# brantburnett/Snappier

Measured on AMD Instinct MI355X. Metric: uncompressed GB/s block compress+decompress, 64 KiB blocks, higher is better.
Workload: dtype u8

## Files before the change

snappier_amd/csrc/capi_internal.h:

```cpp
#pragma once
#include <hip/hip_runtime.h>

#include <cstdio>
#include <cstring>
#include <new>
#include <algorithm>
#include <cmath>
#include <chrono>
#include <mutex>
#include <string>
#include <utility>
#include <vector>

#include "snp_rules.h"

struct ChunkRows {
    u8* type;
    u64 *body_off, *out_off;
    u32 *body_len, *crc, *out_cap, *out_len, *tag;
    i32* status;
};

extern "C" {
hipError_t snp_launch_decompress(const u8*, const u64*, const u32*, u32, u8*, const u64*, const u32*, u32*, i32*,
                                 const u8*, int, hipStream_t, const u32*);
u32 snp_tag_index_entries(u32, u32);
size_t snp_tag_index_workspace_bytes(u32, u32);
size_t snp_tag_index_fallback_offset(u32, u32);
hipError_t snp_launch_tag_index(const u8*, u32, u32, u32, u64*, u64*, u32*, u64*, u32*, u32*, hipStream_t);
u32 snp_tag_index_chunks_ready(u32, u32, u64);
hipError_t snp_launch_tag_index_begin(u64*, u32, u32, int, hipStream_t);
int snp_tag_index_look_back_only(u32, u32);
hipError_t snp_launch_tag_index_chunks(const u8*, u32, u32, u64*, u32, u32, hipStream_t);
hipError_t snp_launch_tag_index_finish(const u8*, u32, u32, u32, u64*, u64*, u32*, u64*, u32*, u32*, hipStream_t);
hipError_t snp_launch_compress_win(const u8*, const u64*, const u32*, u32, u8*, const u64*, u32*, i32*, int, int, int,
                                   hipStream_t, uint16_t*, u32);
size_t snp_compress_win_table_bytes(u32);
hipError_t snp_launch_compress_win_dual(const u8*, const u64*, const u32*, u32, u8*, const u64*, u32*, i32*, int, int, hipStream_t, hipStream_t,
                                        hipEvent_t, hipEvent_t, uint16_t*, u32, u32, u32*);
hipError_t snp_launch_decompress_small(const u8*, const u64*, const u32*, u32, u8*, const u64*, const u32*, u32*, i32*, const u8*,
                                       u32, hipStream_t, u32*, u32*, u32, u32);
hipError_t snp_launch_sample_caps(const u32*, u32, u32, u32*, hipStream_t);
hipError_t snp_launch_decompress_list(const u8*, const u64*, const u32*, u32, u8*, const u64*, const u32*, u32*, i32*, const u8*, int,
                                      hipStream_t, const u32*, u32*, u32, u32);
hipError_t snp_launch_compress_lanes(const u8*, const u64*, const u32*, u32, u8*, const u64*, u32*, i32*, int, int, const snp_table_pieces*,
                                     u32*, hipStream_t, const snp_lane_tuning*);
size_t snp_compress_lanes_workspace(u32);
hipError_t snp_probe_tables(const snp_table_pieces*, u32, u32, hipStream_t, float*);
hipError_t snp_launch_crc32c(const u8*, const u64*, const u32*, u32, int, u32*, const u32*, i32*, hipStream_t);
hipError_t snp_launch_gather(const u8*, const u64*, const u32*, u8*, const u64*, u32, hipStream_t);
hipError_t snp_launch_frame_chunks(u64, u32, u64, u64*, u32*, u64*, hipStream_t);
hipError_t snp_launch_frame_plan(const u32*, const u32*, u32, u8*, u32*, u64*, u64*, hipStream_t);
hipError_t snp_launch_frame_header_only(u8*, u64*, hipStream_t);
hipError_t snp_launch_frame_scan(const u8*, u64, u64, u32, const ChunkRows&, u64*, hipStream_t);
hipError_t snp_launch_frame_result(const i32*, const u64*, u64*, hipStream_t);
size_t snp_frame_scan_workspace(u64);
hipError_t snp_launch_frame_scan_spans(const u8*, u64, u64, u32, const ChunkRows&, u64*, void*, hipStream_t);
hipError_t snp_launch_frame_emit(const u8*, const u64*, const u8*, const u64*, const u8*, const u32*, const u32*,
                                 const u64*, u8*, u64, u32, hipStream_t);
}

constexpr u64 snp_comp_stride(u64 n) { return (38 + n + n / 6 + 15) / 16 * 16 + 16; }
constexpr u64 kSnpCompStride = snp_comp_stride(SNP_BLOCK_SIZE);
static_assert(kSnpCompStride == 76496 + 16, "staging stride of a 64 KiB fragment");

struct DevBuf {
    void* p = nullptr;
    size_t cap = 0;
};

inline u64 snp_align_up(u64 v, u64 a) { return (v + a - 1) / a * a; }

struct TablePool {
    std::mutex mu;
    int users = 0;
    snp_table_pieces tp{};
    void* plain = nullptr;
    size_t plain_cap = 0;
    std::vector<void*> pieces;
    hipEvent_t last_use = nullptr;
    hipStream_t last_stream = nullptr;
    bool used = false;
    bool pinned = false;
    std::vector<void*> retired;
    uint64_t stats[4] = {0, 0, 0, 0};
    void drain();
    void drop_workspace();
    void destroy();
};
TablePool* snp_pool_of(int device);
constexpr int kSnpMaxDevices = 64;

struct RelaxedCaptureMode {
    hipStreamCaptureMode mode = hipStreamCaptureModeRelaxed;
    bool ok;
    RelaxedCaptureMode() { ok = hipThreadExchangeStreamCaptureMode(&mode) == hipSuccess; if (!ok) (void)hipGetLastError(); }
    ~RelaxedCaptureMode() { if (ok && hipThreadExchangeStreamCaptureMode(&mode) != hipSuccess) (void)hipGetLastError(); }
};

struct snp_ctx {
    int device = 0;
    int variant = SNP_HASH_CRC32C;
    hipStream_t stream = nullptr;
    bool own_stream = false;
    int fenced = 0;
    int dec_lds = 0;
    int decode_layout = 0;
    int table_tries = 2;
    uint64_t table_probe_max_bytes = 0;
    u32 par_min = 4 * SNP_BLOCK_SIZE;
    int compress_mode = 0;
    int win_np = 1;
    u32 small_max = 512;
    u32 small_min_blocks = 4096;
    int crc_kernel = 0;
    int crc_bits() const { return crc_kernel == 1 ? 2 : crc_kernel == 2 ? 4 : 0; }
    bool no_prepass = false;
    bool small_lanes = false;
    bool redo_grid = false, redo_list = false;
    u32 small_team_log = 0;
    u32 slice_fragments = 262144;
    u32 win_gtab_min = 4096;
    u32 win_gslots = 0;
    u32 win_dual_min = 1536;
    hipStream_t side_stream = nullptr;
    hipEvent_t side_ev[2] = {nullptr, nullptr};
    int side_state = 0;
    bool side_stream_ready();
    u32 win_max = 32768;
    snp_lane_tuning lane_tune{0, -1, 0, -1, 0, 0};
    DevBuf in, out, meta, work, fragtab, scan, small, redo, win_tables;
    int frame_scan = 0;
    uint64_t counters[7] = {0, 0, 0, 0, 0, 0, 0};
    bool table_tries_set = false;
    std::string err;

    bool launch_decompress(const u8* d_in, const u64* in_off, const u32* in_len, u32 nblocks, u8* d_out, const u64* out_off,
                           const u32* out_cap, u32* out_len, i32* status, const u8* chunk_type);
    bool launch_compress(const u8* d_in, const u64* in_off, const u32* in_len, u32 nblocks, u8* d_out, const u64* out_off,
                         u32* out_len, i32* status, int emit_varint);
    bool decode_chunks(const u8* d_in, const ChunkRows& r, u32 n, u8* d_out);
    u32* hint = nullptr;
    hipEvent_t hint_ev = nullptr;
    bool hint_pending = false, hint_mostly_large = false, hint_from_prepass = false, hint_seen = false;
    u32 hint_blocks = 0, hint_mean_cap = 256;
    bool hint_ready();
    u32 n_waves = 0;
    u32 persistent_waves();
    u32* chint = nullptr;
    hipEvent_t chint_ev = nullptr;
    bool chint_pending = false, chint_small = false, chint_mid = false;
    int chint_tiny = 0;
    bool chint_ready();

    bool check(hipError_t e, const char* what);
    bool ensure(DevBuf& b, size_t bytes, const char* what);
    bool h2d(void* dev, const void* host, size_t n, const char* what);
    bool d2h(void* host, const void* dev, size_t n, const char* what);
    bool stream_is_capturing();
    bool was_captured = false;
    std::vector<void*> kept;
    bool use_device() { return check(hipSetDevice(device), "hipSetDevice"); }
    bool rebind(hipStream_t next);
    hipEvent_t order_ev = nullptr;
    hipStream_t copy_stream = nullptr;
    hipEvent_t copy_ev[2] = {nullptr, nullptr};
    int copy_state = 0;
    bool copy_stream_ready();

    TablePool* pool = nullptr;
    snp_table_pieces tp{};
    bool borrowed = false;
    DevBuf own_tables;
    bool borrow_tables(u32 nblocks, bool thorough = false);
    void return_tables();
    bool build_tables(TablePool& P, u32 nblocks, bool thorough, bool capturing);

    bool upload_and_compress(const u8* host_in, size_t n, u32 nf, const u64* d_in_off, const u32* d_in_len, u8* d_out,
                             const u64* d_out_off, u32* d_out_len, i32* d_status, int emit_varint);
};

struct DevGuard {
    int prev = -1, dev = -1;
    bool ok = false;
    explicit DevGuard(snp_ctx* c) : dev(c->device)
    {
        if (hipGetDevice(&prev) != hipSuccess) prev = -1;
        ok = prev == dev || c->use_device();
        if (ok && !c->was_captured && c->stream) (void)c->stream_is_capturing();
    }
    ~DevGuard() { if (prev >= 0 && prev != dev) (void)hipSetDevice(prev); }
};

snp_status snp_frame_encode_impl(snp_ctx* c, const uint8_t* d_in, const uint8_t* host_in, uint64_t n, uint8_t* d_out, uint64_t cap,
                                 uint64_t* d_written, void* d_work);
inline bool snp_ranges_overlap(const u8* a, size_t an, const u8* b, size_t bn) { return an && bn && a < b + bn && b < a + an; }
```

snappier_amd/csrc/capi_pool.hip:

```cpp
#include "capi_internal.h"
#include "piece_search.h"

using snp_piece_search::PieceSearch;

void TablePool::drain()
{
    RelaxedCaptureMode relaxed;
    if (used && last_use) (void)hipEventSynchronize(last_use);
}

void TablePool::drop_workspace()
{
    drain();
    RelaxedCaptureMode relaxed;
    auto gone = [&](void* q) { if (!q) return; if (pinned) retired.push_back(q); else (void)hipFree(q); };
    gone(plain);
    for (void* q : pieces) gone(q);
    plain = nullptr;
    plain_cap = 0;
    pieces.clear();
    tp = snp_table_pieces{};
}

void TablePool::destroy()
{
    pinned = false;
    drop_workspace();
    for (void* q : retired) (void)hipFree(q);
    retired.clear();
    if (last_use) (void)hipEventDestroy(last_use);
    last_use = nullptr;
    used = false;
}

namespace {
std::mutex g_pools_mu;
}
TablePool* snp_pool_of(int device)
{
    static TablePool* pools[kSnpMaxDevices] = {};
    if (device < 0 || device >= kSnpMaxDevices) return nullptr;
    std::lock_guard<std::mutex> g(g_pools_mu);
    if (!pools[device]) pools[device] = new TablePool();
    return pools[device];
}

bool snp_ctx::borrow_tables(u32 nblocks, bool thorough)
{
    if (table_tries_set && table_tries == 1) {
        const size_t bytes = snp_compress_lanes_workspace(nblocks);
        if (bytes > own_tables.cap) {
            if (stream_is_capturing()) { err = "hash-table workspace: it would have to grow while the stream is being captured"; return false; }
            (void)hipStreamSynchronize(stream);
            if (own_tables.p) { if (was_captured) kept.push_back(own_tables.p); else (void)hipFree(own_tables.p); }
            own_tables = DevBuf{};
            if (!check(hipMalloc(&own_tables.p, bytes + 4096), "hipMalloc(hash tables)")) { own_tables.p = nullptr; return false; }
            own_tables.cap = bytes + 4096;
        }
        tp = snp_table_pieces{};
        tp.p[0] = static_cast<u32*>(own_tables.p);
        tp.piece_frags = 0xffffffc0u;
        tp.n = 1;
        counters[2] = counters[3] = counters[4] = counters[5] = 0;
        return true;
    }
    TablePool& P = *pool;
    P.mu.lock();
    const bool capturing = stream_is_capturing();
    if (!build_tables(P, nblocks, thorough, capturing)) { P.mu.unlock(); return false; }
    if (capturing) {
        P.pinned = true;
    } else if (P.used && P.last_stream != stream) {
        if (!check(hipStreamWaitEvent(stream, P.last_use, 0), "hipStreamWaitEvent(table pool)")) { P.mu.unlock(); return false; }
    }
    tp = P.tp;
    counters[2] = P.stats[0]; counters[3] = P.stats[1]; counters[4] = P.stats[2]; counters[5] = P.stats[3];
    borrowed = true;
    return true;
}

void snp_ctx::return_tables()
{
    if (!borrowed) return;
    TablePool& P = *pool;
    if (!stream_is_capturing()) {
        if (!P.last_use && hipEventCreateWithFlags(&P.last_use, hipEventDisableTiming) != hipSuccess) { (void)hipGetLastError(); P.last_use = nullptr; }
        if (P.last_use && hipEventRecord(P.last_use, stream) == hipSuccess) { P.used = true; P.last_stream = stream; }
        else { (void)hipGetLastError(); (void)hipStreamSynchronize(stream); P.used = false; }
    }
    borrowed = false;
    P.mu.unlock();
}

bool snp_ctx::build_tables(TablePool& P, u32 nblocks, bool thorough, bool capturing)
{
    const size_t bytes = snp_compress_lanes_workspace(nblocks);
    if (!P.pieces.empty() && static_cast<uint64_t>(nblocks) <= static_cast<uint64_t>(P.tp.piece_frags) * P.tp.n) return true;
    if (P.pieces.empty() && P.plain && bytes <= P.plain_cap) return true;
    if (capturing) {
        err = "hash-table workspace: it would have to be built while the stream is being captured -- call snp_ctx_reserve_compress (or make the same call once) before the capture";
        return false;
    }
    RelaxedCaptureMode relaxed;
    const int tries = table_tries_set ? table_tries : 2;
    P.drop_workspace();
    P.stats[0] = P.stats[1] = P.stats[2] = P.stats[3] = 0;
    if (bytes < (1ull << 30) || tries <= 1) {
        const size_t want = bytes >= (1ull << 30) ? bytes + 4096 : bytes + bytes / 4 + 4096;
        if (!check(hipMalloc(&P.plain, want), "hipMalloc(hash tables)")) { P.plain = nullptr; return false; }
        P.plain_cap = want;
        P.tp = snp_table_pieces{};
        P.tp.p[0] = static_cast<u32*>(P.plain);
        P.tp.piece_frags = 0xffffffc0u;
        P.tp.n = 1;
        return true;
    }
    PieceSearch ps{};
    const uint64_t with_slack = static_cast<uint64_t>(nblocks) + nblocks / 16u;
    const u32 cap_frags = static_cast<u32>(with_slack < slice_fragments ? with_slack : (nblocks > slice_fragments ? nblocks : slice_fragments));
    const u32 piece_frags = ((cap_frags + SNP_TABLE_PIECES_MAX - 1) / SNP_TABLE_PIECES_MAX + 63u) / 64u * 64u;
    const size_t piece_bytes = static_cast<size_t>(piece_frags) * 65536u;
    ps.n = (cap_frags + piece_frags - 1) / piece_frags;
    ps.piece_gib = piece_bytes / 1073741824.0;
    ps.max_cand = static_cast<size_t>(ps.n) * static_cast<size_t>(tries);
    ps.dbg = SNP_GETENV("SNAPPIER_HIP_DEBUG") != nullptr;
    if (thorough && table_tries_set) ps.patience = 64;
    size_t free_b = 0, total_b = 0;
    if (hipMemGetInfo(&free_b, &total_b) == hipSuccess) {
        size_t room = free_b / 2;
        if (table_probe_max_bytes) {
            room = static_cast<size_t>(table_probe_max_bytes);
            if (room > free_b / 8 * 7) room = free_b / 8 * 7;
        }
        if (room / piece_bytes < ps.max_cand) ps.max_cand = room / piece_bytes;
    }
    if (ps.max_cand < ps.n) ps.max_cand = ps.n;
    std::vector<u32*> cand;
    ps.alloc_one = [&]() {
        void* q = nullptr;
        if (hipMalloc(&q, piece_bytes) != hipSuccess) { (void)hipGetLastError(); return false; }
        cand.push_back(static_cast<u32*>(q));
        return true;
    };
    ps.probe_set = [&](const std::vector<u32>& pick) {
        snp_table_pieces t{};
        for (size_t i = 0; i < pick.size(); ++i) t.p[i] = cand[pick[i]];
        t.piece_frags = piece_frags;
        t.n = static_cast<u32>(pick.size());
        float ms = 1e30f;
        if (snp_probe_tables(&t, nblocks, 512u, stream, &ms) != hipSuccess) { (void)hipGetLastError(); ms = 1e30f; }
        return ms;
    };
    std::vector<u32> set;
    const auto t_search = std::chrono::steady_clock::now();
    const float ms = ps.run(set);
    if (ms < 0) {
        for (u32* q : cand) (void)hipFree(q);
        err = "hipMalloc(hash tables): out of memory";
        return false;
    }
    std::vector<char> used(cand.size(), 0);
    P.tp = snp_table_pieces{};
    for (u32 i = 0; i < ps.n; ++i) { P.tp.p[i] = cand[set[i]]; used[set[i]] = 1; P.pieces.push_back(cand[set[i]]); }
    P.tp.piece_frags = piece_frags;
    P.tp.n = ps.n;
    for (size_t k = 0; k < cand.size(); ++k)
        if (!used[k]) (void)hipFree(cand[k]);
    P.stats[0] = ms < 1e6f ? static_cast<uint64_t>(ms * 1000.0f) : 0;
    P.stats[1] = static_cast<uint64_t>(cand.size());
    P.stats[2] = static_cast<uint64_t>(std::chrono::duration_cast<std::chrono::microseconds>(std::chrono::steady_clock::now() - t_search).count());
    P.stats[3] = static_cast<uint64_t>(cand.size()) * piece_bytes;
    return true;
}
```

snappier_amd/csrc/compress_lanes.hip:

```cpp
#include <cstdlib>

#include "snp_device.h"

#ifndef SNP_CL_FLAT
#define SNP_CL_FLAT 1
#endif
#ifndef SNP_CL_SLOTS
#define SNP_CL_SLOTS 1
#endif

namespace {

constexpr u32 kDefaultSlots = SNP_CL_SLOTS;

constexpr u32 crc_step32(u32 x)
{
    for (int k = 0; k < 32; ++k) x = (x >> 1) ^ ((x & 1u) ? 0x82F63B78u : 0u);
    return x;
}

__device__ __forceinline__ u32 check_bits(u32 bytes) { return (bytes * 0x9E3779B1u) & 0xffff0000u; }

__device__ __forceinline__ u32 table_swap(u32* p, u32 v) { return __hip_atomic_exchange(p, v, __ATOMIC_RELAXED, __HIP_MEMORY_SCOPE_AGENT); }

struct LaneCtx {
    const u8* src;
    u8* dst;
    u32* table;
    u32 first4;
    u32 n;
    u32 mask;
    u32 hmask;
};

template <int VARIANT>
__device__ __forceinline__ u32 lane_hash(const LaneCtx& c, u32 bytes, const u16 (*lut)[256])
{
    u32 hash;
    if constexpr (VARIANT == SNP_HASH_CRC32C) {
        hash = lut[0][bytes & 0xffu] ^ lut[1][(bytes >> 8) & 0xffu] ^ lut[2][(bytes >> 16) & 0xffu] ^ lut[3][bytes >> 24] ^ c.hmask;
    } else {
        hash = (0x1e35a7bdu * bytes) >> 17;
    }
    return (hash & c.mask) >> 1;
}

__device__ __forceinline__ u32 lane_emit_literal(const LaneCtx& c, u32 op, u32 s, u32 len)
{
    u8* o = c.dst + op;
    const u32 k = len - 1;
    u32 hdr;
    if (k < 60) { o[0] = static_cast<u8>(k << 2); hdr = 1; }
    else if (k < 256) { o[0] = static_cast<u8>(60u << 2); o[1] = static_cast<u8>(k); hdr = 2; }
    else { o[0] = static_cast<u8>(61u << 2); o[1] = static_cast<u8>(k); o[2] = static_cast<u8>(k >> 8); hdr = 3; }
    const u8* src = c.src + s;
    u8* d = o + hdr;
    u32 i = 0;
    for (; i + 16 <= len; i += 16)
        *reinterpret_cast<snp_u128_unaligned*>(d + i) = *reinterpret_cast<const snp_u128_unaligned*>(src + i);
    for (; i + 4 <= len; i += 4) st32u(d + i, ld32u(src + i));
    for (; i < len; ++i) d[i] = src[i];
    return op + hdr + len;
}

__device__ __forceinline__ u32 lane_emit_literal16(const LaneCtx& c, u32 op, u32 s, u32 len, const snp_u128_unaligned& first, u32 cap, bool merge)
{
    u8* o = c.dst + op;
    const u32 k = len - 1;
    if (merge && len <= 15 && op + 16 <= cap) {
        snp_u128_unaligned w;
        w.v[0] = (first.v[0] << 8) | (k << 2);
        w.v[1] = __builtin_amdgcn_alignbit(first.v[1], first.v[0], 24);
        w.v[2] = __builtin_amdgcn_alignbit(first.v[2], first.v[1], 24);
        w.v[3] = __builtin_amdgcn_alignbit(first.v[3], first.v[2], 24);
        *reinterpret_cast<snp_u128_unaligned*>(o) = w;
        return op + 1 + len;
    }
    u32 hdr;
    if (k < 60) { o[0] = static_cast<u8>(k << 2); hdr = 1; }
    else if (k < 256) { o[0] = static_cast<u8>(60u << 2); o[1] = static_cast<u8>(k); hdr = 2; }
    else { o[0] = static_cast<u8>(61u << 2); o[1] = static_cast<u8>(k); o[2] = static_cast<u8>(k >> 8); hdr = 3; }
    u8* d = o + hdr;
    if (len >= 16 || op + hdr + 16 <= cap) {
        *reinterpret_cast<snp_u128_unaligned*>(d) = first;
    } else {
        u32 w[4] = {first.v[0], first.v[1], first.v[2], first.v[3]};
        u32 at = 0, wi = 0;
        if (len & 8) { st32u(d, w[0]); st32u(d + 4, w[1]); at = 8; wi = 2; }
        if (len & 4) { st32u(d + at, w[wi]); at += 4; ++wi; }
        u32 rest = w[wi & 3];
        if (len & 2) { d[at] = static_cast<u8>(rest); d[at + 1] = static_cast<u8>(rest >> 8); rest >>= 16; at += 2; }
        if (len & 1) d[at] = static_cast<u8>(rest);
    }
    if (len > 16) {
        const u8* src = c.src + s;
        u32 i = 16;
        for (; i + 16 <= len; i += 16)
            *reinterpret_cast<snp_u128_unaligned*>(d + i) = *reinterpret_cast<const snp_u128_unaligned*>(src + i);
        if (i < len)
            *reinterpret_cast<snp_u128_unaligned*>(d + len - 16) = *reinterpret_cast<const snp_u128_unaligned*>(src + len - 16);
    }
    return op + hdr + len;
}

__device__ __forceinline__ u32 lane_emit_copy64(u8* dst, u32 op, u32 off, u32 len, u32 cap)
{
    u8* o = dst + op;
    const bool one = len < 12 && off < 2048;
    const u32 w = one ? (1u | ((len - 4) << 2) | ((off >> 8) << 5) | ((off & 0xffu) << 8)) : (2u | ((len - 1) << 2) | (off << 8));
    if (op + 4 <= cap) {
        st32u(o, w);
    } else {
        o[0] = static_cast<u8>(w);
        o[1] = static_cast<u8>(w >> 8);
        if (!one) o[2] = static_cast<u8>(w >> 16);
    }
    return op + (one ? 2u : 3u);
}

__device__ __forceinline__ u32 lane_emit_copy(u8* dst, u32 op, u32 off, u32 len, u32 cap = 0)
{
    while (len >= 68) { op = lane_emit_copy64(dst, op, off, 64, cap); len -= 64; }
    if (len > 64) { op = lane_emit_copy64(dst, op, off, 60, cap); len -= 60; }
    return lane_emit_copy64(dst, op, off, len, cap);
}

__device__ __forceinline__ u32 lane_find_match_length(const u8* src, u32 s1, u32 s2, u32 n)
{
    u32 matched = 0;
    while (s2 + matched + 8 <= n) {
        const u64 x = ld64u(src + s1 + matched) ^ ld64u(src + s2 + matched);
        if (x) return matched + (static_cast<u32>(__builtin_ctzll(x)) >> 3);
        matched += 8;
    }
    while (s2 + matched < n && src[s1 + matched] == src[s2 + matched]) ++matched;
    return matched;
}

constexpr u32 kStageStride = 100;

struct OutStage {
    u8* lds;
    u32 flushed;
};

__device__ __forceinline__ void stage_flush64(const LaneCtx& c, OutStage& st)
{
    u8* g = c.dst + st.flushed;
    typedef u32 v4u __attribute__((ext_vector_type(4), aligned(1)));
#pragma unroll
    for (u32 i = 0; i < 64; i += 16) {
        const snp_u128_unaligned q = *reinterpret_cast<const snp_u128_unaligned*>(st.lds + i);
        const v4u v = {q.v[0], q.v[1], q.v[2], q.v[3]};
        __builtin_nontemporal_store(v, reinterpret_cast<v4u*>(g + i));
    }
    const snp_u128_unaligned t0 = *reinterpret_cast<const snp_u128_unaligned*>(st.lds + 64);
    const snp_u128_unaligned t1 = *reinterpret_cast<const snp_u128_unaligned*>(st.lds + 80);
    *reinterpret_cast<snp_u128_unaligned*>(st.lds) = t0;
    *reinterpret_cast<snp_u128_unaligned*>(st.lds + 16) = t1;
    st.flushed += 64;
}

__device__ __forceinline__ void stage_drain(const LaneCtx& c, OutStage& st, u32 op)
{
    const u32 fill = op - st.flushed;
    u8* g = c.dst + st.flushed;
    u32 i = 0;
    for (; i + 16 <= fill; i += 16)
        *reinterpret_cast<snp_u128_unaligned*>(g + i) = *reinterpret_cast<const snp_u128_unaligned*>(st.lds + i);
    for (; i < fill; ++i) g[i] = st.lds[i];
    st.flushed = op;
}

enum : int {
    kOptBlindLiterals = 1,
    kOptBlindLiteral16 = 2,
    kOptBlindCopies = 4,
    kOptShortExtend = 8,
    kOptStagedOutput = 16,
    kOptExchangeProbe = 64,
    kOptInputWindow = 128,
};

template <int VARIANT, u32 kSlots, bool SMALL>
__global__ __launch_bounds__(SNP_WAVE) void k_compress_lanes(const u8* __restrict__ in, const u64* __restrict__ in_off,
                                                            const u32* __restrict__ in_len, u32 nblocks,
                                                            u8* __restrict__ out, const u64* __restrict__ out_off,
                                                            u32* __restrict__ out_len, i32* __restrict__ status,
                                                            int emit_varint, const snp_table_pieces tp, int opts,
                                                            const u32* __restrict__ max_len, u32 small_max)
{
    __shared__ u16 lut[4][256];
    if (VARIANT == SNP_HASH_CRC32C) {
        for (u32 e = threadIdx.x; e < 1024; e += blockDim.x)
            lut[e >> 8][e & 255u] = static_cast<u16>(crc_step32((e & 255u) << (8 * (e >> 8))) & 0x7ffeu);
        __syncthreads();
    }
    __shared__ u8 s_out[SMALL ? 16 : SNP_WAVE * kStageStride];
    const u32 b = blockIdx.x * blockDim.x + threadIdx.x;
    const u32 maxlen = *max_len;
    if (SMALL ? maxlen > small_max : (small_max != 0 && maxlen <= small_max)) return;
    extern __shared__ __attribute__((aligned(16))) u8 s_dyn[];
    const u32 tstride = maxlen > 16384 ? 16384u : maxlen < 256 ? 256u : (2u << (31u - __clz(maxlen - 1)));
    u32* wt;
    {
        const u32 first = blockIdx.x * blockDim.x;
        const u32 mine = nblocks - first < blockDim.x ? nblocks - first : blockDim.x;
        const u32 piece = first / tp.piece_frags;
        wt = tp.p[piece] + static_cast<size_t>(first - piece * tp.piece_frags) * tstride;
        const size_t words = static_cast<size_t>(mine) * tstride;
        if (tstride == 16384u) {
            typedef u32 v4u __attribute__((ext_vector_type(4)));
            const v4u zero4 = {0, 0, 0, 0};
            for (size_t i = static_cast<size_t>(threadIdx.x) * 4; i < words; i += static_cast<size_t>(blockDim.x) * 4)
                __builtin_nontemporal_store(zero4, reinterpret_cast<v4u*>(wt + i));
        } else {
            for (size_t i = static_cast<size_t>(threadIdx.x) * 4; i < words; i += static_cast<size_t>(blockDim.x) * 4)
                *reinterpret_cast<uint4*>(wt + i) = make_uint4(0, 0, 0, 0);
        }
        asm volatile("s_waitcnt vmcnt(0)" ::: "memory");
    }
    if (b >= nblocks) return;
    const bool staged = (opts & kOptStagedOutput) != 0;
    const bool t_swap = kSlots == 1 && (opts & kOptExchangeProbe) != 0;
    bool in_win = (opts & kOptInputWindow) != 0;
    OutStage stg{(SMALL ? s_dyn + blockDim.x * (small_max + 16u) : s_out) + threadIdx.x * kStageStride, 0};

    LaneCtx c;
    c.dst = out + out_off[b];
    c.n = in_len[b];
    c.table = wt + static_cast<size_t>(threadIdx.x) * tstride;
    const u32 n = c.n;
    if constexpr (SMALL) {
        const u8* g = in + in_off[b];
        u8* mine = s_dyn + threadIdx.x * (small_max + 16u);
        u32 i = 0;
        for (; i + 16 <= n; i += 16) {
            const snp_u128_unaligned q = *reinterpret_cast<const snp_u128_unaligned*>(g + i);
            *reinterpret_cast<uint4*>(mine + i) = make_uint4(q.v[0], q.v[1], q.v[2], q.v[3]);
        }
        for (; i + 4 <= n; i += 4) *reinterpret_cast<u32*>(mine + i) = ld32u(g + i);
        for (; i < n; ++i) mine[i] = g[i];
        c.src = mine;
    } else {
        c.src = in + in_off[b];
    }
    c.first4 = n >= 4 ? ld32u(c.src) : 0u;
    if (n > SNP_BLOCK_SIZE) { out_len[b] = 0; status[b] = SNP_ERR_BAD_ARG; return; }

    u32 op = 0;
    if (emit_varint) {
        u32 v = n;
        while (v >= 128) { c.dst[op++] = static_cast<u8>(v | 0x80u); v >>= 7; }
        c.dst[op++] = static_cast<u8>(v);
    }
    stg.flushed = op;

    u32 ip = 0;
#if SNP_CL_FLAT
    enum : u32 { kScan = 0, kPost = 1, kExtend = 2, kDone = 3 };
    u32 mode = kDone;
    u32 next_emit = 0, skip = 32, cand = 0, base = 0, mlen = 0, limit = 0;
    snp_u128_unaligned win = {};
    u32 win_at = 0x80000000u;
    in_win = in_win && n >= 32;
    if (n >= 15) {
        const u32 tsize = n > 16384 ? 16384u : n < 256 ? 256u : (2u << (31u - __clz(n - 1)));
        c.mask = 2 * (tsize - 1);
        c.hmask = static_cast<u16>(crc_step32(c.mask) & 0x7ffeu);
        limit = n - 15;
        mode = kScan;
        ip = 1;
    }
    const u32 lit_cap = (opts & kOptBlindLiterals) ? 32u + n + n / 6u : 0u;
    while (__any(mode != kDone)) {
        u32 cp_len = 0, cp_off = 0;
        u32 lit_len = 0;
        snp_u128_unaligned lit16 = {};
        const bool post = mode == kPost;
        const bool scanning = mode == kScan || post;
        u32 p[kSlots], nx[kSlots], sk[kSlots], d[kSlots], h[kSlots], cv[kSlots];
        bool legal[kSlots];
        u64 w0 = 0;
        if (scanning) {
            u32 q = ip, sv = skip;
            bool ok = true;
#pragma unroll
            for (u32 k = 0; k < kSlots; ++k) {
                const u32 bb = post ? 0u : sv >> 5;
                sv += bb;
                p[k] = q;
                nx[k] = q + bb;
                sk[k] = sv;
                ok = ok && (post ? k == 0 : nx[k] <= limit);
                legal[k] = ok;
                q = nx[k];
            }
            const u32 at = ip - (post ? 1u : 0u);
            if (in_win) {
                u32 o = at - win_at;
                if (o > 8u) {
                    win_at = min(at, n - 16u);
                    win = *reinterpret_cast<const snp_u128_unaligned*>(c.src + win_at);
                    o = at - win_at;
                }
                const u32 dq = o >> 2, sh = (o & 3u) * 8u;
                const u32 a0 = dq == 0 ? win.v[0] : dq == 1 ? win.v[1] : win.v[2];
                const u32 a1 = dq == 0 ? win.v[1] : dq == 1 ? win.v[2] : win.v[3];
                const u32 a2 = dq == 0 ? win.v[2] : dq == 1 ? win.v[3] : 0u;
                const u64 lo = (static_cast<u64>(a1) << 32) | a0;
                w0 = sh ? (lo >> sh) | (static_cast<u64>(a2) << (64u - sh)) : lo;
            } else {
                w0 = ld64u(c.src + at);
            }
        } else {
#pragma unroll
            for (u32 k = 0; k < kSlots; ++k) { p[k] = nx[k] = sk[k] = 0; legal[k] = false; }
        }
        const bool ext = mode == kExtend;
        const bool ext_wide = ext && base + mlen + 32 <= n;
        snp_u128_unaligned xa0 = {}, xa1 = {}, xb0 = {}, xb1 = {};
        if (ext_wide) {
            const u8* a = c.src + cand + mlen;
            const u8* bq = c.src + base + mlen;
            xa0 = *reinterpret_cast<const snp_u128_unaligned*>(a);
            xb0 = *reinterpret_cast<const snp_u128_unaligned*>(bq);
            if (!(opts & kOptShortExtend)) {
                xa1 = *reinterpret_cast<const snp_u128_unaligned*>(a + 16);
                xb1 = *reinterpret_cast<const snp_u128_unaligned*>(bq + 16);
            }
        }
        u32 hm1 = ~0u, vm1 = 0;
        bool swapped = false;
        if (scanning) {
            if (post) {
                const u32 dm1 = static_cast<u32>(w0);
                hm1 = lane_hash<VARIANT>(c, dm1, lut);
                vm1 = (ip - 1) | check_bits(dm1);
                if (tstride == 16384u) __builtin_nontemporal_store(vm1, &c.table[hm1]);
                else c.table[hm1] = vm1;
                d[0] = static_cast<u32>(w0 >> 8);
            } else {
                d[0] = static_cast<u32>(w0);
            }
#pragma unroll
            for (u32 k = 1; k < kSlots; ++k) {
                d[k] = 0;
                if (legal[k]) {
                    const u32 delta = p[k] - p[0];
                    d[k] = delta <= 4 ? static_cast<u32>(w0 >> (8 * delta)) : ld32u(c.src + p[k]);
                }
            }
#pragma unroll
            for (u32 k = 0; k < kSlots; ++k) h[k] = lane_hash<VARIANT>(c, d[k], lut);
            if (t_swap) {
                swapped = legal[0] && h[0] != hm1;
                cv[0] = !legal[0] ? 0u : swapped ? table_swap(&c.table[h[0]], p[0] | check_bits(d[0])) : vm1;
            } else {
#pragma unroll
                for (u32 k = 0; k < kSlots; ++k) cv[k] = legal[k] ? c.table[h[k]] : 0u;
            }
        }
        if (ext) {
            bool finished = false;
            if (ext_wide) {
                const u64 x0 = (static_cast<u64>(xa0.v[0] ^ xb0.v[0])) | (static_cast<u64>(xa0.v[1] ^ xb0.v[1]) << 32);
                const u64 x1 = (static_cast<u64>(xa0.v[2] ^ xb0.v[2])) | (static_cast<u64>(xa0.v[3] ^ xb0.v[3]) << 32);
                const u64 x2 = (static_cast<u64>(xa1.v[0] ^ xb1.v[0])) | (static_cast<u64>(xa1.v[1] ^ xb1.v[1]) << 32);
                const u64 x3 = (static_cast<u64>(xa1.v[2] ^ xb1.v[2])) | (static_cast<u64>(xa1.v[3] ^ xb1.v[3]) << 32);
                finished = true;
                if (x0) mlen += static_cast<u32>(__builtin_ctzll(x0)) >> 3;
                else if (x1) mlen += 8 + (static_cast<u32>(__builtin_ctzll(x1)) >> 3);
                else if (opts & kOptShortExtend) { mlen += 16; finished = false; }
                else if (x2) mlen += 16 + (static_cast<u32>(__builtin_ctzll(x2)) >> 3);
                else if (x3) mlen += 24 + (static_cast<u32>(__builtin_ctzll(x3)) >> 3);
                else { mlen += 32; finished = false; }
            } else {
                for (u32 k = 0; k < 4 && !finished; ++k) {
                    if (base + mlen + 8 <= n) {
                        const u64 x = ld64u(c.src + cand + mlen) ^ ld64u(c.src + base + mlen);
                        if (x) { mlen += static_cast<u32>(__builtin_ctzll(x)) >> 3; finished = true; }
                        else mlen += 8;
                    } else {
                        while (base + mlen < n && c.src[cand + mlen] == c.src[base + mlen]) ++mlen;
                        finished = true;
                    }
                }
            }
            if (finished) {
                ip = base + mlen;
                cp_len = mlen;
                cp_off = base - cand;
                mode = ip >= limit ? kDone : kPost;
            }
        }
        if (scanning) {
#pragma unroll
            for (u32 k = 1; k < kSlots; ++k)
#pragma unroll
                for (u32 i = 0; i < k; ++i)
                    if (legal[k] && h[i] == h[k]) cv[k] = p[i] | check_bits(d[i]);
            u32 kw = kSlots;
#pragma unroll
            for (u32 k = kSlots; k-- > 0;) {
                const u32 pos = cv[k] & 0xffffu;
                const bool want = legal[k] && (pos == 0 ? c.first4 == d[k] : (cv[k] & 0xffff0000u) == check_bits(d[k]));
                if (want) kw = k;
            }
            u32 wp = 0, wpos = 0;
#pragma unroll
            for (u32 k = 0; k < kSlots; ++k)
                if (kw == k) { wp = p[k]; wpos = cv[k] & 0xffffu; }
            snp_u128_unaligned cb = {}, pb = {}, lb = {};
            if (kw < kSlots) {
                cb = *reinterpret_cast<const snp_u128_unaligned*>(c.src + wpos);
                pb = *reinterpret_cast<const snp_u128_unaligned*>(c.src + wp);
                if (!post) lb = *reinterpret_cast<const snp_u128_unaligned*>(c.src + next_emit);
            }
            bool ended = false;
#pragma unroll
            for (u32 k = 0; k < kSlots; ++k) {
                if (!ended && k <= kw) {
                    if (!legal[k]) {
                        if (!post) { ended = true; ip = next_emit; mode = kDone; }
                    } else if (!swapped) {
                        c.table[h[k]] = p[k] | check_bits(d[k]);
                    }
                }
            }
            if (!ended) {
                bool hit = false;
                if (kw < kSlots) {
                    const u64 x0 = (static_cast<u64>(cb.v[0] ^ pb.v[0])) | (static_cast<u64>(cb.v[1] ^ pb.v[1]) << 32);
                    const u64 x1 = (static_cast<u64>(cb.v[2] ^ pb.v[2])) | (static_cast<u64>(cb.v[3] ^ pb.v[3]) << 32);
                    hit = static_cast<u32>(x0) == 0;
                    if (hit) {
                        if (!post) {
                            if (staged) { lit_len = wp - next_emit; lit16 = lb; }
                            else op = lane_emit_literal16(c, op, next_emit, wp - next_emit, lb, lit_cap, (opts & kOptBlindLiteral16) != 0);
                        }
                        base = wp;
                        cand = wpos;
                        if (x0) mlen = static_cast<u32>(__builtin_ctzll(x0)) >> 3;
                        else if (x1) mlen = 8 + (static_cast<u32>(__builtin_ctzll(x1)) >> 3);
                        else mlen = 16;
                        if (mlen < 16) {
                            ip = base + mlen;
                            cp_len = mlen;
                            cp_off = base - cand;
                            mode = ip >= limit ? kDone : kPost;
                        } else {
                            mode = kExtend;
                        }
                    }
                }
                if (!hit) {
                    if (post) {
                        next_emit = ip;
                        ++ip;
                        skip = 32;
                        mode = kScan;
                    } else {
                        const u32 last = kw < kSlots ? kw : kSlots - 1;
#pragma unroll
                        for (u32 k = 0; k < kSlots; ++k)
                            if (k == last) { ip = nx[k]; skip = sk[k]; }
                    }
                }
            }
        }
        if (!staged) {
            if (cp_len) op = lane_emit_copy(c.dst, op, cp_off, cp_len, (opts & kOptBlindCopies) ? lit_cap : 0u);
        } else {
            if (lit_len) {
                if (lit_len <= 15) {
                    snp_u128_unaligned w;
                    w.v[0] = (lit16.v[0] << 8) | ((lit_len - 1) << 2);
                    w.v[1] = __builtin_amdgcn_alignbit(lit16.v[1], lit16.v[0], 24);
                    w.v[2] = __builtin_amdgcn_alignbit(lit16.v[2], lit16.v[1], 24);
                    w.v[3] = __builtin_amdgcn_alignbit(lit16.v[3], lit16.v[2], 24);
                    *reinterpret_cast<snp_u128_unaligned*>(stg.lds + (op - stg.flushed)) = w;
                    op += 1 + lit_len;
                } else {
                    stage_drain(c, stg, op);
                    op = lane_emit_literal16(c, op, next_emit, lit_len, lit16, 0u, false);
                    stg.flushed = op;
                }
            }
            u32 len = cp_len;
            while (len) {
                const u32 piece = len >= 68 ? 64u : len > 64 ? 60u : len;
                const bool one = piece < 12 && cp_off < 2048;
                const u32 w = one ? (1u | ((piece - 4) << 2) | ((cp_off >> 8) << 5) | ((cp_off & 0xffu) << 8))
                                  : (2u | ((piece - 1) << 2) | (cp_off << 8));
                st32u(stg.lds + (op - stg.flushed), w);
                op += one ? 2u : 3u;
                len -= piece;
                if (op - stg.flushed >= 64) stage_flush64(c, stg);
            }
            if (op - stg.flushed >= 64) stage_flush64(c, stg);
        }
    }
    if (staged) stage_drain(c, stg, op);
#else
    if (n >= 15) {
        const u32 tsize = n > 16384 ? 16384u : n < 256 ? 256u : (2u << (31u - __clz(n - 1)));
        c.mask = 2 * (tsize - 1);
        c.hmask = static_cast<u16>(crc_step32(c.mask) & 0x7ffeu);
        const u32 limit = n - 15;
        for (;;) {
            const u32 next_emit = ip;
            ++ip;
            u32 skip = 32;
            u32 cand;
            for (;;) {
                const u32 data = ld32u(c.src + ip);
                const u32 bb = skip >> 5;
                skip += bb;
                const u32 nxt = ip + bb;
                if (nxt > limit) { ip = next_emit; goto emit_remainder; }
                const u32 h = lane_hash<VARIANT>(c, data, lut);
                cand = c.table[h] & 0xffffu;
                c.table[h] = ip | check_bits(data);
                if (ld32u(c.src + cand) == data) break;
                ip = nxt;
            }
            op = lane_emit_literal(c, op, next_emit, ip - next_emit);
            for (;;) {
                const u32 base = ip;
                const u32 matched = 4 + lane_find_match_length(c.src, cand + 4, ip + 4, n);
                ip += matched;
                op = lane_emit_copy(c.dst, op, base - cand, matched);
                if (ip >= limit) goto emit_remainder;
                const u32 dm1 = ld32u(c.src + ip - 1);
                c.table[lane_hash<VARIANT>(c, dm1, lut)] = (ip - 1) | check_bits(dm1);
                const u32 data = ld32u(c.src + ip);
                const u32 h = lane_hash<VARIANT>(c, data, lut);
                cand = c.table[h] & 0xffffu;
                c.table[h] = ip | check_bits(data);
                if (ld32u(c.src + cand) != data) break;
            }
        }
    }
emit_remainder:
#endif
    if (ip < n) op = lane_emit_literal(c, op, ip, n - ip);
    out_len[b] = op;
    status[b] = SNP_OK;
}

}

namespace {
__global__ __launch_bounds__(SNP_WAVE) void k_probe_tables(const snp_table_pieces tp, u32 nblocks, u32 probes)
{
    const u32 g = blockIdx.x * SNP_WAVE + threadIdx.x;
    if (g >= nblocks) return;
    u32* t = tp.p[(g / tp.piece_frags) % tp.n] + static_cast<size_t>(g % tp.piece_frags) * 16384u;
    u32 st = g * 2654435761u + 1u;
    for (u32 i = 0; i < probes; ++i) {
        const u32 h = (st * 0x1e35a7bdu) >> 18;
        const u32 v = table_swap(&t[h], i);
        st = st * 1664525u + 1013904223u + v;
    }
    if (st == 0x12345678u) tp.p[0][0] = st;
}
}

extern "C" hipError_t snp_probe_tables(const snp_table_pieces* tp, u32 nblocks, u32 probes, hipStream_t stream, float* ms)
{
    hipEvent_t a, b;
    hipError_t e = hipEventCreate(&a);
    if (e != hipSuccess) return e;
    e = hipEventCreate(&b);
    if (e != hipSuccess) { (void)hipEventDestroy(a); return e; }
    const u32 grid = (nblocks + SNP_WAVE - 1) / SNP_WAVE;
    hipLaunchKernelGGL(k_probe_tables, dim3(grid), dim3(SNP_WAVE), 0, stream, *tp, nblocks, 64u);
    (void)hipEventRecord(a, stream);
    hipLaunchKernelGGL(k_probe_tables, dim3(grid), dim3(SNP_WAVE), 0, stream, *tp, nblocks, probes);
    (void)hipEventRecord(b, stream);
    e = hipEventSynchronize(b);
    if (e == hipSuccess) e = hipEventElapsedTime(ms, a, b);
    (void)hipEventDestroy(a);
    (void)hipEventDestroy(b);
    return e;
}

namespace {
__global__ void k_debug_lane_match_length(const u8* buf, u32 n, u32 s1, u32 s2, u32* out)
{
    if (threadIdx.x == 0) *out = lane_find_match_length(buf, s1, s2, n);
}
}
extern "C" int snp_debug_lane_match_length(const u8* d_buf, u32 n, u32 s1, u32 s2, u32* d_out, hipStream_t stream)
{
    hipLaunchKernelGGL(k_debug_lane_match_length, dim3(1), dim3(SNP_WAVE), 0, stream, d_buf, n, s1, s2, d_out);
    return static_cast<int>(hipGetLastError());
}

extern "C" size_t snp_compress_lanes_workspace(u32 nblocks) { return static_cast<size_t>(nblocks) * 16384u * sizeof(u32); }

__global__ __launch_bounds__(256) void k_max_len(const u32* __restrict__ in_len, u32 nblocks, u32* __restrict__ max_len)
{
    u32 m = 0;
    for (u32 i = blockIdx.x * 256 + threadIdx.x; i < nblocks; i += gridDim.x * 256) m = max(m, in_len[i]);
    for (int sh = 32; sh >= 1; sh >>= 1) m = max(m, static_cast<u32>(__shfl_xor(static_cast<int>(m), sh, 64)));
    if ((threadIdx.x & 63u) == 0) atomicMax(max_len, m);
}

extern "C" hipError_t snp_launch_compress_lanes(const u8* in, const u64* in_off, const u32* in_len, u32 nblocks, u8* out,
                                                const u64* out_off, u32* out_len, i32* status, int variant,
                                                int emit_varint, const snp_table_pieces* tables, u32* max_len, hipStream_t stream, const snp_lane_tuning* tune)
{
    if (nblocks == 0) return hipSuccess;
    hipError_t e = snp_zero_words_async(max_len, 1, stream);
    if (e != hipSuccess) return e;
    const u32 mgrid = (nblocks + 255) / 256 < 1024 ? (nblocks + 255) / 256 : 1024u;
    hipLaunchKernelGGL(k_max_len, dim3(mgrid), dim3(256), 0, stream, in_len, nblocks, max_len);
    const char* env = SNP_GETENV("SNAPPIER_HIP_LANES_PER_WAVE");
    const bool two_probes = (tune->hint & 256) != 0;
    const u32 small_hint = ((static_cast<u32>(tune->hint) >> 9) & 63u) << 4;
    const u32 lanes_hint = tune->lanes_per_wave ? static_cast<u32>(tune->lanes_per_wave) : static_cast<u32>(tune->hint & 255);
    u32 per = env ? static_cast<u32>(atoi(env)) : lanes_hint ? lanes_hint : (nblocks >= 131072 ? 64u : nblocks >= 8192 ? 32u : 16u);
    if (per != 64 && per != 32 && per != 16 && per != 8) per = 64;
    const u32 grid = (nblocks + per - 1) / per;
    const char* ex = SNP_GETENV("SNAPPIER_HIP_EXACT_LITERALS");
    const char* oe = SNP_GETENV("SNAPPIER_HIP_CL_OPTS");
    const int opts = ((ex && ex[0] == '1') ? 0 : oe ? (atoi(oe) & 255) : tune->opts >= 0 ? (tune->opts & 255)
                      : ((nblocks >= 32768 ? 23 : 7) | 64 | ((nblocks >= 131072 && !two_probes) ? 128 : 0)));
    const char* se = SNP_GETENV("SNAPPIER_HIP_CL_SLOTS");
    const u32 slots = se ? static_cast<u32>(atoi(se)) : tune->probes > 0 ? static_cast<u32>(tune->probes) : ((nblocks >= 131072 && !two_probes) ? kDefaultSlots : 2u);
    const char* sm = SNP_GETENV("SNAPPIER_HIP_CL_SMALL");
    u32 small_max = sm ? (static_cast<u32>(atoi(sm)) + 15u) & ~15u : tune->small_bytes >= 0 ? (static_cast<u32>(tune->small_bytes) + 15u) & ~15u : small_hint;
    if (small_max > 2048) small_max = 0;
    if (small_max) {
        const char* sp = SNP_GETENV("SNAPPIER_HIP_CL_SMALL_PER");
        u32 sper = sp ? static_cast<u32>(atoi(sp)) : tune->small_lanes ? static_cast<u32>(tune->small_lanes) : 32u;
        if (sper != 64 && sper != 32 && sper != 16) sper = 32;
        const u32 sgrid = (nblocks + sper - 1) / sper;
        const u32 dyn = sper * (small_max + 16u + kStageStride);
        bool small_ok = true;
#define SNP_LAUNCH_SMALL(V)                                                                                                                         \
    do {                                                                                                                                            \
        if (dyn > 48u * 1024u && hipFuncSetAttribute(reinterpret_cast<const void*>(&k_compress_lanes<V, 2, true>), hipFuncAttributeMaxDynamicSharedMemorySize, static_cast<int>(dyn)) != hipSuccess) { \
            small_ok = false;                                                                                                                       \
            break;                                                                                                                                  \
        }                                                                                                                                           \
        hipLaunchKernelGGL((k_compress_lanes<V, 2, true>), dim3(sgrid), dim3(sper), dyn, stream, in, in_off, in_len, nblocks, out, out_off, out_len, status, \
                           emit_varint, *tables, opts, max_len, small_max);                                                                    \
        small_ok = hipGetLastError() == hipSuccess;                                                                                                 \
    } while (0)
        if (variant == SNP_HASH_CRC32C) SNP_LAUNCH_SMALL(SNP_HASH_CRC32C); else SNP_LAUNCH_SMALL(SNP_HASH_MUL);
#undef SNP_LAUNCH_SMALL
        if (!small_ok) {
            (void)hipGetLastError();
            small_max = 0;
        }
    }
#define SNP_LAUNCH_CL(V, S)                                                                                          \
    hipLaunchKernelGGL((k_compress_lanes<V, S, false>), dim3(grid), dim3(per), 0, stream, in, in_off, in_len, nblocks, out,    \
                       out_off, out_len, status, emit_varint, *tables, opts, max_len, small_max)
    if (variant == SNP_HASH_CRC32C) { if (slots == 1) SNP_LAUNCH_CL(SNP_HASH_CRC32C, 1); else if (slots >= 4) SNP_LAUNCH_CL(SNP_HASH_CRC32C, 4); else if (slots == 3) SNP_LAUNCH_CL(SNP_HASH_CRC32C, 3); else SNP_LAUNCH_CL(SNP_HASH_CRC32C, 2); }
    else { if (slots == 1) SNP_LAUNCH_CL(SNP_HASH_MUL, 1); else if (slots >= 4) SNP_LAUNCH_CL(SNP_HASH_MUL, 4); else if (slots == 3) SNP_LAUNCH_CL(SNP_HASH_MUL, 3); else SNP_LAUNCH_CL(SNP_HASH_MUL, 2); }
#undef SNP_LAUNCH_CL
    return hipGetLastError();
}
```

snappier_amd/csrc/snp_device.h:

```cpp
#pragma once
#include <hip/hip_runtime.h>
#include <stdint.h>

#include "../../include/snappier_hip.h"

typedef uint8_t u8;
typedef uint16_t u16;
typedef uint32_t u32;
typedef uint64_t u64;
typedef int32_t i32;

#define SNP_WAVE 64
#define SNP_SCAN_TILE 1024u

#ifdef SNAPPIER_HIP_DEBUG_ENV
#include <stdlib.h>
#define SNP_GETENV(name) getenv(name)
#else
#define SNP_GETENV(name) static_cast<const char*>(nullptr)
#endif

#define SNP_TABLE_PIECES_MAX 16
struct snp_table_pieces {
    uint32_t* p[SNP_TABLE_PIECES_MAX];
    uint32_t piece_frags;
    uint32_t n;
};

struct snp_lane_tuning {
    int lanes_per_wave;
    int opts;
    int probes;
    int small_bytes;
    int small_lanes;
    int hint;
};

struct __attribute__((packed)) snp_u32_unaligned { u32 v; };
struct __attribute__((packed)) snp_u64_unaligned { u64 v; };
struct __attribute__((packed)) snp_u128_unaligned { u32 v[4]; };

__device__ __forceinline__ u32 ld32u(const u8* p) { return reinterpret_cast<const snp_u32_unaligned*>(p)->v; }
__device__ __forceinline__ u64 ld64u(const u8* p) { return reinterpret_cast<const snp_u64_unaligned*>(p)->v; }
__device__ __forceinline__ void st32u(u8* p, u32 v) { reinterpret_cast<snp_u32_unaligned*>(p)->v = v; }

__device__ __forceinline__ u32 lane_id() { return __builtin_amdgcn_mbcnt_hi(~0u, __builtin_amdgcn_mbcnt_lo(~0u, 0u)); }
__device__ __forceinline__ u64 ballot64(bool p) { return __ballot(p); }
__device__ __forceinline__ u32 bcast_first(u32 v) { return __builtin_amdgcn_readfirstlane(v); }
__device__ __forceinline__ u32 read_lane(u32 v, u32 lane) { return __builtin_amdgcn_readlane(v, lane); }
__device__ __forceinline__ u64 lanes_below(u32 lane) { return lane >= 64 ? ~0ull : ((1ull << lane) - 1ull); }

__device__ __forceinline__ u64 wave_min(u64 v)
{
    for (u32 d = 32; d >= 1; d >>= 1) {
        const u64 o = __shfl_xor(v, d, 64);
        v = o < v ? o : v;
    }
    return v;
}
__device__ __forceinline__ u64 wave_max(u64 v)
{
    for (u32 d = 32; d >= 1; d >>= 1) {
        const u64 o = __shfl_xor(v, d, 64);
        v = o > v ? o : v;
    }
    return v;
}
__device__ __forceinline__ u64 wave_sum(u64 v)
{
    for (u32 d = 32; d >= 1; d >>= 1) v += __shfl_xor(v, d, 64);
    return v;
}
__device__ __forceinline__ void atomic_min64(u64* p, u64 v) { atomicMin(reinterpret_cast<unsigned long long*>(p), static_cast<unsigned long long>(v)); }
__device__ __forceinline__ void atomic_max64(u64* p, u64 v) { atomicMax(reinterpret_cast<unsigned long long*>(p), static_cast<unsigned long long>(v)); }
__device__ __forceinline__ void atomic_add64(u64* p, u64 v) { atomicAdd(reinterpret_cast<unsigned long long*>(p), static_cast<unsigned long long>(v)); }

__device__ __forceinline__ void wave_copy(u8* dst, const u8* src, u32 len, u32 lane)
{
    u32 done = 0;
    while (len - done >= 1024) {
        snp_u128_unaligned w = *reinterpret_cast<const snp_u128_unaligned*>(src + done + lane * 16);
        *reinterpret_cast<snp_u128_unaligned*>(dst + done + lane * 16) = w;
        done += 1024;
    }
    while (len - done >= 256) {
        st32u(dst + done + lane * 4, ld32u(src + done + lane * 4));
        done += 256;
    }
#pragma clang loop vectorize(disable) unroll(disable)
    for (u32 k = done + lane; k < len; k += 64) dst[k] = src[k];
}

__device__ __forceinline__ void block_copy(u8* dst, const u8* src, u32 len, u32 tid)
{
    u32 k = tid * 16;
    for (; k + 16 <= len; k += 256 * 16) {
        snp_u128_unaligned w = *reinterpret_cast<const snp_u128_unaligned*>(src + k);
        *reinterpret_cast<snp_u128_unaligned*>(dst + k) = w;
    }
    const u32 tail = len & ~15u;
    if (tid < (len & 15u)) dst[tail + tid] = src[tail + tid];
}

__host__ __device__ __forceinline__ u32 crc32c_mask(u32 x) { return ((x >> 15) | (x << 17)) + 0xa282ead8u; }

namespace {
__global__ void k_zero_words(u32* p, u32 n)
{
    for (u32 i = threadIdx.x; i < n; i += blockDim.x) p[i] = 0u;
}
}
static inline hipError_t snp_zero_words_async(u32* p, u32 n, hipStream_t stream)
{
    hipLaunchKernelGGL(k_zero_words, dim3(1), dim3(64), 0, stream, p, n);
    return hipGetLastError();
}
```

Measured before the change: 101.2.

## Use epoch-tagged hash tables to skip per-call table zeroing

Adds a per-fragment generation byte array and packs a 4-bit epoch into each hash table entry, shrinking the check bits from 16 to 12. Each call bumps the fragment's epoch, so stale entries from earlier calls are treated as empty and the 64 KiB table is wiped only when the epoch wraps. This removes most of the per-call nontemporal zeroing traffic of the 16384-entry tables. In exchange it adds a generation read/write per block, costs 4 check bits (more false candidates to verify), and adds extra allocations and memsets for the generation bytes.

```diff
diff --git a/snappier_amd/csrc/capi_internal.h b/snappier_amd/csrc/capi_internal.h
--- a/snappier_amd/csrc/capi_internal.h
+++ b/snappier_amd/csrc/capi_internal.h
@@ -78,6 +78,7 @@
     void* plain = nullptr;
     size_t plain_cap = 0;
     std::vector<void*> pieces;
+    void* gen = nullptr;
     hipEvent_t last_use = nullptr;
     hipStream_t last_stream = nullptr;
     bool used = false;
@@ -86,6 +87,7 @@
     uint64_t stats[4] = {0, 0, 0, 0};
     void drain();
     void drop_workspace();
+    bool reset_generations(size_t slots, hipStream_t stream);
     void destroy();
 };
 TablePool* snp_pool_of(int device);
diff --git a/snappier_amd/csrc/capi_pool.hip b/snappier_amd/csrc/capi_pool.hip
--- a/snappier_amd/csrc/capi_pool.hip
+++ b/snappier_amd/csrc/capi_pool.hip
@@ -16,10 +16,20 @@
     auto gone = [&](void* q) { if (!q) return; if (pinned) retired.push_back(q); else (void)hipFree(q); };
     gone(plain);
     for (void* q : pieces) gone(q);
+    gone(gen);
+    gen = nullptr;
     plain = nullptr;
     plain_cap = 0;
     pieces.clear();
     tp = snp_table_pieces{};
+}
+
+bool TablePool::reset_generations(size_t slots, hipStream_t stream)
+{
+    if (hipMalloc(&gen, slots) != hipSuccess) { (void)hipGetLastError(); gen = nullptr; return false; }
+    if (hipMemsetAsync(gen, static_cast<int>(SNP_GEN_UNKNOWN), slots, stream) != hipSuccess) { (void)hipGetLastError(); return false; }
+    tp.gen = static_cast<u8*>(gen);
+    return true;
 }
 
 void TablePool::destroy()
@@ -54,11 +64,18 @@
             (void)hipStreamSynchronize(stream);
             if (own_tables.p) { if (was_captured) kept.push_back(own_tables.p); else (void)hipFree(own_tables.p); }
             own_tables = DevBuf{};
-            if (!check(hipMalloc(&own_tables.p, bytes + 4096), "hipMalloc(hash tables)")) { own_tables.p = nullptr; return false; }
+            const size_t slots = static_cast<size_t>(nblocks) + 64;
+            if (!check(hipMalloc(&own_tables.p, bytes + 4096 + slots), "hipMalloc(hash tables)")) { own_tables.p = nullptr; return false; }
             own_tables.cap = bytes + 4096;
+            if (!check(hipMemsetAsync(static_cast<u8*>(own_tables.p) + own_tables.cap, static_cast<int>(SNP_GEN_UNKNOWN), slots, stream), "hipMemsetAsync(table generations)")) {
+                (void)hipFree(own_tables.p);
+                own_tables = DevBuf{};
+                return false;
+            }
         }
         tp = snp_table_pieces{};
         tp.p[0] = static_cast<u32*>(own_tables.p);
+        tp.gen = static_cast<u8*>(own_tables.p) + own_tables.cap;
         tp.piece_frags = 0xffffffc0u;
         tp.n = 1;
         counters[2] = counters[3] = counters[4] = counters[5] = 0;
@@ -113,6 +130,7 @@
         P.tp.p[0] = static_cast<u32*>(P.plain);
         P.tp.piece_frags = 0xffffffc0u;
         P.tp.n = 1;
+        if (!P.reset_generations(want / 65536u + 64, stream)) { P.drop_workspace(); err = "hipMalloc(table generations) failed"; return false; }
         return true;
     }
     PieceSearch ps{};
@@ -166,6 +184,7 @@
     P.tp.n = ps.n;
     for (size_t k = 0; k < cand.size(); ++k)
         if (!used[k]) (void)hipFree(cand[k]);
+    if (!P.reset_generations(static_cast<size_t>(piece_frags) * ps.n, stream)) { P.drop_workspace(); err = "hipMalloc(table generations) failed"; return false; }
     P.stats[0] = ms < 1e6f ? static_cast<uint64_t>(ms * 1000.0f) : 0;
     P.stats[1] = static_cast<uint64_t>(cand.size());
     P.stats[2] = static_cast<uint64_t>(std::chrono::duration_cast<std::chrono::microseconds>(std::chrono::steady_clock::now() - t_search).count());
diff --git a/snappier_amd/csrc/compress_lanes.hip b/snappier_amd/csrc/compress_lanes.hip
--- a/snappier_amd/csrc/compress_lanes.hip
+++ b/snappier_amd/csrc/compress_lanes.hip
@@ -19,7 +19,9 @@
     return x;
 }
 
-__device__ __forceinline__ u32 check_bits(u32 bytes) { return (bytes * 0x9E3779B1u) & 0xffff0000u; }
+__device__ __forceinline__ u32 check_bits(u32 bytes) { return (bytes * 0x9E3779B1u) & 0xfff00000u; }
+constexpr u32 kCheckMask = 0xfff00000u, kEpochMask = 0x000f0000u;
+__device__ __forceinline__ u32 entry_pos(u32 entry, u32 etag) { return ((entry ^ etag) & kEpochMask) ? 0u : entry & 0xffffu; }
 
 __device__ __forceinline__ u32 table_swap(u32* p, u32 v) { return __hip_atomic_exchange(p, v, __ATOMIC_RELAXED, __HIP_MEMORY_SCOPE_AGENT); }
 
@@ -31,7 +33,9 @@
     u32 n;
     u32 mask;
     u32 hmask;
+    u32 etag;
 };
+__device__ __forceinline__ u32 make_entry(const LaneCtx& c, u32 pos, u32 bytes) { return pos | c.etag | check_bits(bytes); }
 
 template <int VARIANT>
 __device__ __forceinline__ u32 lane_hash(const LaneCtx& c, u32 bytes, const u16 (*lut)[256])
@@ -178,9 +182,11 @@
     kOptBlindCopies = 4,
     kOptShortExtend = 8,
     kOptStagedOutput = 16,
+    kOptEpochTables = 32,
     kOptExchangeProbe = 64,
     kOptInputWindow = 128,
 };
+constexpr int kAutoEpochTables = kOptEpochTables;
 
 template <int VARIANT, u32 kSlots, bool SMALL>
 __global__ __launch_bounds__(SNP_WAVE) void k_compress_lanes(const u8* __restrict__ in, const u64* __restrict__ in_off,
@@ -203,13 +209,29 @@
     extern __shared__ __attribute__((aligned(16))) u8 s_dyn[];
     const u32 tstride = maxlen > 16384 ? 16384u : maxlen < 256 ? 256u : (2u << (31u - __clz(maxlen - 1)));
     u32* wt;
+    u32 epoch = 0;
     {
         const u32 first = blockIdx.x * blockDim.x;
         const u32 mine = nblocks - first < blockDim.x ? nblocks - first : blockDim.x;
         const u32 piece = first / tp.piece_frags;
         wt = tp.p[piece] + static_cast<size_t>(first - piece * tp.piece_frags) * tstride;
         const size_t words = static_cast<size_t>(mine) * tstride;
-        if (tstride == 16384u) {
+        if (tstride == 16384u && (opts & kOptEpochTables)) {
+            bool wipe = false;
+            if (b < nblocks) {
+                const u32 g = tp.gen[b];
+                wipe = g >= 15u;
+                epoch = g == SNP_GEN_UNKNOWN ? 1u + b % 15u : wipe ? 1u : g + 1u;
+                tp.gen[b] = static_cast<u8>(epoch);
+            }
+            typedef u32 v4u __attribute__((ext_vector_type(4)));
+            const v4u zero4 = {0, 0, 0, 0};
+            for (u64 m = ballot64(wipe); m; m &= m - 1) {
+                u32* t = wt + static_cast<size_t>(__builtin_ctzll(m)) * 16384u;
+                for (u32 i = threadIdx.x * 4; i < 16384u; i += blockDim.x * 4)
+                    __builtin_nontemporal_store(zero4, reinterpret_cast<v4u*>(t + i));
+            }
+        } else if (tstride == 16384u) {
             typedef u32 v4u __attribute__((ext_vector_type(4)));
             const v4u zero4 = {0, 0, 0, 0};
             for (size_t i = static_cast<size_t>(threadIdx.x) * 4; i < words; i += static_cast<size_t>(blockDim.x) * 4)
@@ -230,6 +252,7 @@
     c.dst = out + out_off[b];
     c.n = in_len[b];
     c.table = wt + static_cast<size_t>(threadIdx.x) * tstride;
+    c.etag = epoch << 16;
     const u32 n = c.n;
     if constexpr (SMALL) {
         const u8* g = in + in_off[b];
@@ -336,7 +359,7 @@
             if (post) {
                 const u32 dm1 = static_cast<u32>(w0);
                 hm1 = lane_hash<VARIANT>(c, dm1, lut);
-                vm1 = (ip - 1) | check_bits(dm1);
+                vm1 = make_entry(c, ip - 1, dm1);
                 if (tstride == 16384u) __builtin_nontemporal_store(vm1, &c.table[hm1]);
                 else c.table[hm1] = vm1;
                 d[0] = static_cast<u32>(w0 >> 8);
@@ -355,7 +378,7 @@
             for (u32 k = 0; k < kSlots; ++k) h[k] = lane_hash<VARIANT>(c, d[k], lut);
             if (t_swap) {
                 swapped = legal[0] && h[0] != hm1;
-                cv[0] = !legal[0] ? 0u : swapped ? table_swap(&c.table[h[0]], p[0] | check_bits(d[0])) : vm1;
+                cv[0] = !legal[0] ? 0u : swapped ? table_swap(&c.table[h[0]], make_entry(c, p[0], d[0])) : vm1;
             } else {
 #pragma unroll
                 for (u32 k = 0; k < kSlots; ++k) cv[k] = legal[k] ? c.table[h[k]] : 0u;
@@ -399,18 +422,18 @@
             for (u32 k = 1; k < kSlots; ++k)
 #pragma unroll
                 for (u32 i = 0; i < k; ++i)
-                    if (legal[k] && h[i] == h[k]) cv[k] = p[i] | check_bits(d[i]);
+                    if (legal[k] && h[i] == h[k]) cv[k] = make_entry(c, p[i], d[i]);
             u32 kw = kSlots;
 #pragma unroll
             for (u32 k = kSlots; k-- > 0;) {
-                const u32 pos = cv[k] & 0xffffu;
-                const bool want = legal[k] && (pos == 0 ? c.first4 == d[k] : (cv[k] & 0xffff0000u) == check_bits(d[k]));
+                const u32 pos = entry_pos(cv[k], c.etag);
+                const bool want = legal[k] && (pos == 0 ? c.first4 == d[k] : (cv[k] & kCheckMask) == check_bits(d[k]));
                 if (want) kw = k;
             }
             u32 wp = 0, wpos = 0;
 #pragma unroll
             for (u32 k = 0; k < kSlots; ++k)
-                if (kw == k) { wp = p[k]; wpos = cv[k] & 0xffffu; }
+                if (kw == k) { wp = p[k]; wpos = entry_pos(cv[k], c.etag); }
             snp_u128_unaligned cb = {}, pb = {}, lb = {};
             if (kw < kSlots) {
                 cb = *reinterpret_cast<const snp_u128_unaligned*>(c.src + wpos);
@@ -424,7 +447,7 @@
                     if (!legal[k]) {
                         if (!post) { ended = true; ip = next_emit; mode = kDone; }
                     } else if (!swapped) {
-                        c.table[h[k]] = p[k] | check_bits(d[k]);
+                        c.table[h[k]] = make_entry(c, p[k], d[k]);
                     }
                 }
             }
@@ -520,8 +543,8 @@
                 const u32 nxt = ip + bb;
                 if (nxt > limit) { ip = next_emit; goto emit_remainder; }
                 const u32 h = lane_hash<VARIANT>(c, data, lut);
-                cand = c.table[h] & 0xffffu;
-                c.table[h] = ip | check_bits(data);
+                cand = entry_pos(c.table[h], c.etag);
+                c.table[h] = make_entry(c, ip, data);
                 if (ld32u(c.src + cand) == data) break;
                 ip = nxt;
             }
@@ -533,11 +556,11 @@
                 op = lane_emit_copy(c.dst, op, base - cand, matched);
                 if (ip >= limit) goto emit_remainder;
                 const u32 dm1 = ld32u(c.src + ip - 1);
-                c.table[lane_hash<VARIANT>(c, dm1, lut)] = (ip - 1) | check_bits(dm1);
+                c.table[lane_hash<VARIANT>(c, dm1, lut)] = make_entry(c, ip - 1, dm1);
                 const u32 data = ld32u(c.src + ip);
                 const u32 h = lane_hash<VARIANT>(c, data, lut);
-                cand = c.table[h] & 0xffffu;
-                c.table[h] = ip | check_bits(data);
+                cand = entry_pos(c.table[h], c.etag);
+                c.table[h] = make_entry(c, ip, data);
                 if (ld32u(c.src + cand) != data) break;
             }
         }
@@ -626,8 +649,9 @@
     const u32 grid = (nblocks + per - 1) / per;
     const char* ex = SNP_GETENV("SNAPPIER_HIP_EXACT_LITERALS");
     const char* oe = SNP_GETENV("SNAPPIER_HIP_CL_OPTS");
-    const int opts = ((ex && ex[0] == '1') ? 0 : oe ? (atoi(oe) & 255) : tune->opts >= 0 ? (tune->opts & 255)
-                      : ((nblocks >= 32768 ? 23 : 7) | 64 | ((nblocks >= 131072 && !two_probes) ? 128 : 0)));
+    int opts = ((ex && ex[0] == '1') ? 0 : oe ? (atoi(oe) & 255) : tune->opts >= 0 ? (tune->opts & 255)
+                : ((nblocks >= 32768 ? 23 : 7) | 64 | ((nblocks >= 131072 && !two_probes) ? 128 : 0) | kAutoEpochTables));
+    if (!tables->gen) opts &= ~static_cast<int>(kOptEpochTables);
     const char* se = SNP_GETENV("SNAPPIER_HIP_CL_SLOTS");
     const u32 slots = se ? static_cast<u32>(atoi(se)) : tune->probes > 0 ? static_cast<u32>(tune->probes) : ((nblocks >= 131072 && !two_probes) ? kDefaultSlots : 2u);
     const char* sm = SNP_GETENV("SNAPPIER_HIP_CL_SMALL");
diff --git a/snappier_amd/csrc/snp_device.h b/snappier_amd/csrc/snp_device.h
--- a/snappier_amd/csrc/snp_device.h
+++ b/snappier_amd/csrc/snp_device.h
@@ -25,7 +25,9 @@
     uint32_t* p[SNP_TABLE_PIECES_MAX];
     uint32_t piece_frags;
     uint32_t n;
+    uint8_t* gen;
 };
+#define SNP_GEN_UNKNOWN 0xffu
 
 struct snp_lane_tuning {
     int lanes_per_wave;
```

Result: faster. 102.5, median of 6 (+1.3%).
